# haberdashPI/SignalOperators.jl

Hardware: NVIDIA B200
Metric: sink Msamples/s (Filt+resample+Mix chain) at 1/2/4/8 B200; % of HBM peak (higher is better)
Workload: dtype f64

## Files before the change

signaloperators.jl_b200/csrc/k_fir_tmap.cuh:

```cuda
#pragma once
#include <cuda.h>

#include <type_traits>

#include "k_fir_mma.cuh"

namespace sigops {

constexpr int kFtRows = 128;
constexpr int kFtSlotPos = 16;
constexpr int kFtSlotBytes = kFtRows * 128;
constexpr int kFtMaxSlots = 10;
constexpr int kFtNCW = 8, kFtNAW = 4;
constexpr int kFtThreads = 16 * 32;
constexpr int kFtRegsCompute = 176, kFtRegsHelper = 112, kFtRegsMisc = 40;
constexpr int kFtMaxKs = 64;

struct FirTmParams {
    double* scalars;
    int nscalars, sumsq_slot, nch;
    int64_t nrows, n_out;
    int tapsper;
    int ks;
    int nslot;
    int64_t ntiles, tiles_per_seg;
    const double* pfb;
    const double* dpfb;
    const int64_t* xi0;
    const int32_t* poff;
    const double* alpha;
    int tab_doubles;
    double gain;
    const double* bands_g;
    int period_tiles;
    int64_t epoch_tiles;
    int n_epochs;
    long long* dbg;
    int exp;
};

inline size_t fir_tm_smem_bytes(int nslot, int ks, int tab_doubles, bool has_dpfb) {
    return (size_t)nslot * kFtSlotBytes + 2 * 16384 + (size_t)2 * 4 * ks * 8 * sizeof(double) +
           (size_t)tab_doubles * sizeof(double) * (has_dpfb ? 2 : 1) + 1024;
}

__device__ __forceinline__ void tmap_load_2d(unsigned smem_dst, const CUtensorMap* tm, int c0, int c1, uint64_t* bar) {
    asm volatile("cp.async.bulk.tensor.2d.shared::cluster.global.mbarrier::complete_tx::bytes [%0], [%1, {%2, %3}], [%4];" ::"r"(smem_dst),
                 "l"(tm), "r"(c0), "r"(c1), "r"(smem_u32(bar))
                 : "memory");
}
__device__ __forceinline__ void tmap_store_2d(const CUtensorMap* tm, int c0, int c1, unsigned smem_src) {
    asm volatile("cp.async.bulk.tensor.2d.global.shared::cta.bulk_group [%0, {%1, %2}], [%3];" ::"l"(tm), "r"(c0), "r"(c1), "r"(smem_src)
                 : "memory");
}
__device__ __forceinline__ double lds_f64(unsigned a) {
    double v;
    asm volatile("ld.shared.f64 %0, [%1];" : "=d"(v) : "r"(a));
    return v;
}
__device__ __forceinline__ void sts_f64(unsigned a, double v) { asm volatile("st.shared.f64 [%0], %1;" ::"r"(a), "d"(v) : "memory"); }
__device__ __forceinline__ void sts_v2f64(unsigned a, double x, double y) {
    asm volatile("st.shared.v2.f64 [%0], {%1, %2};" ::"r"(a), "d"(x), "d"(y) : "memory");
}

__device__ __forceinline__ void mbar_wait_a(unsigned bar, unsigned parity) {
    asm volatile(
        "{\n"
        ".reg .pred p;\n"
        "LAB_WAIT:\n"
        "mbarrier.try_wait.parity.shared::cta.b64 p, [%0], %1;\n"
        "@p bra LAB_DONE;\n"
        "bra LAB_WAIT;\n"
        "LAB_DONE:\n"
        "}\n" ::"r"(bar), "r"(parity) : "memory");
}
__device__ __forceinline__ void mbar_arrive_a(unsigned bar) {
    asm volatile("mbarrier.arrive.shared::cta.b64 _, [%0];" ::"r"(bar) : "memory");
}

template <bool SSQ, bool DBG = false>
__global__ void __launch_bounds__(kFtThreads, 1)
k_fir_tmap(const __grid_constant__ FirTmParams P, const __grid_constant__ CUtensorMap tm_in,
           const __grid_constant__ CUtensorMap tm_out) {
    extern __shared__ unsigned char ft_smem_raw[];
    __shared__ uint64_t bar_full[kFtMaxSlots], bar_done[4], bar_taps[2], bar_stg_full[2], bar_stg_free[2];
    __shared__ unsigned done_count;

    const unsigned ring = (smem_u32(ft_smem_raw) + 1023u) & ~1023u;
    const unsigned stg = ring + (unsigned)P.nslot * kFtSlotBytes;
    const unsigned bands = stg + 2 * 16384;
    const unsigned tabs = bands + 2u * 4u * (unsigned)P.ks * 64u;

    const int tid = threadIdx.x, warp = tid >> 5, lane = tid & 31;
    const int row0 = (int)blockIdx.y * kFtRows;
    const int64_t t0 = (int64_t)blockIdx.x * P.tiles_per_seg;
    const int64_t t1 = (t0 + P.tiles_per_seg < P.ntiles) ? t0 + P.tiles_per_seg : P.ntiles;
    if (t0 >= t1) return;

    for (int i = tid; i < P.tab_doubles; i += kFtThreads) {
        sts_f64(tabs + 8u * i, __ldg(P.pfb + i) * P.gain);
        if (P.dpfb) sts_f64(tabs + 8u * (P.tab_doubles + i), __ldg(P.dpfb + i) * P.gain);
    }
    if (tid == 0) {
        done_count = 0u;
        for (int i = 0; i < P.nslot; ++i) mbar_init(&bar_full[i], 1);
        for (int i = 0; i < 4; ++i) mbar_init(&bar_done[i], kFtNCW);
        mbar_init(&bar_taps[0], P.bands_g ? 2 : kFtNAW * 32);
        mbar_init(&bar_taps[1], P.bands_g ? 2 : kFtNAW * 32);
        for (int i = 0; i < 2; ++i) {
            mbar_init(&bar_stg_full[i], kFtNCW / 2);
            mbar_init(&bar_stg_free[i], 1);
        }
        asm volatile("fence.mbarrier_init.release.cluster;" ::: "memory");
    }
    fence_async_smem();
    __syncthreads();

    const int64_t pos_base = (__ldg(P.xi0 + t0 * kFmT) - P.tapsper + 1) & ~int64_t(kFtSlotPos - 1);
    const unsigned band_tile = 4u * (unsigned)P.ks * 64u;

    if (warp < kFtNCW) {
        constexpr int F = 8;
        const int gw = warp & 3, rw = warp >> 2;
        asm volatile("setmaxnreg.inc.sync.aligned.u32 %0;" ::"n"(kFtRegsCompute));
        const int kk = lane & 3, rr = lane >> 2;
        const int rmap = ((rr & 1) << 2) | (rr & 2) | (rr >> 2);
        const int rloc = rw * (8 * F) + rmap;
        const int nn = rr ^ ((kk >> 1) << 2);
        unsigned key = (unsigned)rmap << 4;
        unsigned srow = stg + rloc * 128;
        unsigned bcol = (unsigned)((gw * P.ks + kk) * 64 + nn * 8);
        unsigned arow1 = ring + rloc * 128;
        unsigned ring_end = arow1 + (unsigned)P.nslot * kFtSlotBytes;
        unsigned a_taps = smem_u32(&bar_taps[0]), a_free = smem_u32(&bar_stg_free[rw]), a_full = smem_u32(&bar_stg_full[rw]);
        unsigned a_done = smem_u32(&bar_done[0]), a_cnt = smem_u32(&done_count), lead = lane == 0 ? 1u : 0u;
        asm volatile("" : "+r"(key), "+r"(srow), "+r"(bcol), "+r"(arow1), "+r"(ring_end));
        asm volatile("" : "+r"(a_taps), "+r"(a_free), "+r"(a_full), "+r"(a_done), "+r"(a_cnt), "+r"(lead));
        const int nt = (int)(t1 - t0);
        const int64_t* xp = P.xi0 + t0 * kFmT + 8 * gw;
        double ssq[SSQ ? 8 : 1];
#pragma unroll
        for (int i = 0; i < (SSQ ? 8 : 1); ++i) ssq[i] = 0.0;

        int64_t xq_nx, x7_nx;
        auto fetch_idx = [&](int u) {
            xq_nx = __ldg(xp + (int64_t)u * kFmT);
            x7_nx = __ldg(xp + (int64_t)u * kFmT + 7);
        };
        fetch_idx(0);
        long long dbg_acc[5] = {0, 0, 0, 0, 0};

        unsigned cur = arow1, nxt = arow1;
        int jcur = 0;
        unsigned off[4];
        bool w[4];
        unsigned bq = 0;
        int nbt = 0;
        struct Ops { double a[F], b; };
        Ops o0, o1;

        auto load_ops = [&](Ops& o, auto J) {
            const unsigned ap = (w[J.value] ? nxt : cur) + off[J.value];
#pragma unroll
            for (int i = 0; i < F; ++i) o.a[i] = lds_f64(ap + i * 1024);
            o.b = lds_f64(bq);
            bq += 256;
        };
        auto next_slot = [&]() {
            ++jcur;
            cur = nxt;
            nxt += kFtSlotBytes;
            if (nxt == ring_end) nxt = arow1;
        };
        auto setup = [&](int u, Ops& o) {
            const long long cs = DBG ? clock64() : 0;
            const int s = u & 1;
            const int r = (int)(xq_nx - P.tapsper + 1 - pos_base) + kk;
            int n = (int)(x7_nx - xq_nx) + P.tapsper + 3;
            n >>= 2;
            nbt = n < (P.ks >> 2) ? n : (P.ks >> 2);
            if (u + 1 < nt) fetch_idx(u + 1);
            const int j_new = r >> 4;
            int slot = (int)((cur - arow1) / kFtSlotBytes) + (j_new - jcur);
            while (slot >= P.nslot) slot -= P.nslot;
            while (slot < 0) slot += P.nslot;
            jcur = j_new;
            cur = arow1 + (unsigned)slot * kFtSlotBytes;
            nxt = cur + kFtSlotBytes;
            if (nxt == ring_end) nxt = arow1;
            const unsigned sub0 = (unsigned)(r & 15) << 3;
#pragma unroll
            for (int J = 0; J < 4; ++J) {
                const unsigned q = sub0 + 32u * J;
                w[J] = q >= 128u;
                off[J] = (q & 127u) ^ key;
            }
            bq = bands + s * band_tile + bcol;
            const long long c0 = DBG ? clock64() : 0;
            if (!(P.exp & 16)) mbar_wait_a(a_taps + 8u * s, (unsigned)(u >> 1) & 1u);
            if (DBG) dbg_acc[0] += clock64() - c0;
            load_ops(o, std::integral_constant<int, 0>{});
            if (DBG) dbg_acc[1] += clock64() - cs;
        };
        auto mma_block = [&](double (&acc)[F][2], const Ops& o) {
#pragma unroll
            for (int i = 0; i < F; ++i) dmma884(acc[i][0], acc[i][1], o.a[i], o.b);
        };
        auto stage_store = [&](double (&o)[F][2], int u_old) {
            const long long c0 = DBG ? clock64() : 0;
            if (u_old > 0) mbar_wait_a(a_free, (unsigned)(u_old - 1) & 1u);
            if (DBG) dbg_acc[2] += clock64() - c0;
            if (!(P.exp & 1)) {
                const unsigned sp = srow + (gw >> 1) * 16384 + ((unsigned)(((gw & 1) * 4 + kk) << 4) ^ key);
#pragma unroll
                for (int i = 0; i < F; ++i) sts_v2f64(sp + i * 1024, o[i][0], o[i][1]);
            }
            if (SSQ) {
#pragma unroll
                for (int i = 0; i < F; ++i) ssq[i] = fma(o[i][0], o[i][0], fma(o[i][1], o[i][1], ssq[i]));
            }
            if (DBG) dbg_acc[3] += clock64() - c0;
        };
        auto stage_signal = [&]() {
            const long long c0 = DBG ? clock64() : 0;
            fence_async_smem();
            __syncwarp();
            if (lead) mbar_arrive_a(a_full);
            if (DBG) dbg_acc[3] += clock64() - c0;
        };
        auto tile = [&](double (&acc)[F][2], double (&old)[F][2], int u) {
            const bool more = u + 1 < nt;
#pragma unroll
            for (int i = 0; i < F; ++i) acc[i][0] = acc[i][1] = 0.0;
            const int n = nbt;
            using I0 = std::integral_constant<int, 0>;
            using I1 = std::integral_constant<int, 1>;
            using I2 = std::integral_constant<int, 2>;
            using I3 = std::integral_constant<int, 3>;
            int b = 0;
            bool signalled = u == 0;
            while (true) {
                if (b + 1 < n) {
                    load_ops(o1, I1{});
                    mma_block(acc, o0);
                    if (b == 0 && u > 0) stage_store(old, u - 1);
                } else {
                    if (more) setup(u + 1, o1);
                    mma_block(acc, o0);
                    if (b == 0 && u > 0) stage_store(old, u - 1);
                    o0 = o1;
                    break;
                }
                ++b;
                if (b + 1 < n) {
                    load_ops(o0, I2{});
                    mma_block(acc, o1);
                } else {
                    if (more) setup(u + 1, o0);
                    mma_block(acc, o1);
                    break;
                }
                ++b;
                if (b + 1 < n) {
                    load_ops(o1, I3{});
                    mma_block(acc, o0);
                    if (b == 2 && u > 0) { stage_signal(); signalled = true; }
                } else {
                    if (more) setup(u + 1, o1);
                    mma_block(acc, o0);
                    o0 = o1;
                    break;
                }
                ++b;
                if (b + 1 < n) {
                    next_slot();
                    load_ops(o0, I0{});
                    mma_block(acc, o1);
                } else {
                    if (more) setup(u + 1, o0);
                    mma_block(acc, o1);
                    break;
                }
                ++b;
            }
            if (!signalled) stage_signal();
            __syncwarp();
            if (lead) {
                mbar_arrive_a(a_done + 8u * (u & 3));
                asm volatile("red.release.cta.shared::cta.add.u32 [%0], 1;" ::"r"(a_cnt) : "memory");
            }
        };

        double accA[F][2], accB[F][2];
        setup(0, o0);
        const long long cstart = DBG ? clock64() : 0;
        for (int u = 0; u < nt; u += 2) {
            tile(accA, accB, u);
            if (u + 1 < nt) tile(accB, accA, u + 1);
        }
        if (DBG && warp == 0 && lane == 0) {
            long long* d = P.dbg + ((size_t)blockIdx.y * gridDim.x + blockIdx.x) * 8;
            d[0] = dbg_acc[0]; d[1] = dbg_acc[1]; d[2] = dbg_acc[2]; d[3] = clock64() - cstart; d[6] = dbg_acc[3];
        }
        if (nt & 1) stage_store(accA, nt - 1);
        else stage_store(accB, nt - 1);
        stage_signal();
        if (SSQ) {
#pragma unroll
            for (int i = 0; i < F; ++i) {
                double v = ssq[i];
                v += __shfl_xor_sync(0xffffffffu, v, 1);
                v += __shfl_xor_sync(0xffffffffu, v, 2);
                const int64_t row = (int64_t)row0 + rloc + 8 * i;
                if (kk == 0 && row < P.nrows) atomicAdd(P.scalars + (size_t)(row / P.nch) * P.nscalars + P.sumsq_slot, v);
            }
        }
    } else if (warp < kFtNCW + kFtNAW) {
        asm volatile("setmaxnreg.dec.sync.aligned.u32 %0;" ::"n"(kFtRegsHelper));
        const int grp = warp - kFtNCW;
        if (P.bands_g) {
            if (grp == 0 && lane == 0) {
                const unsigned bytes = 4u * (unsigned)P.ks * 64u;
                int64_t jwait = 0;
                int jw_slot = 0;
                unsigned jw_par = 0;
                for (int64_t t = t0; t < t1; ++t) {
                    const int64_t u = t - t0;
                    const int s = (int)(u & 1);
                    const int64_t hi = (__ldg(P.xi0 + t * kFmT + kFmT - 1) + 4 - pos_base + (kFtSlotPos - 1)) >> 4;
                    if (u >= 2) mbar_wait(&bar_done[(u - 2) & 3], (unsigned)((u - 2) >> 2) & 1u);
                    mbar_expect_tx(&bar_taps[s], bytes);
                    int64_t ep = t / P.epoch_tiles;
                    ep = ep < P.n_epochs ? ep : P.n_epochs - 1;
                    const double* src = P.bands_g + (size_t)(ep * P.period_tiles + t % P.period_tiles) * (bytes / 8);
                    asm volatile("cp.async.bulk.shared::cluster.global.mbarrier::complete_tx::bytes [%0], [%1], %2, [%3];" ::"r"(
                                     bands + (unsigned)s * band_tile),
                                 "l"(src), "r"(bytes), "r"(smem_u32(&bar_taps[s]))
                                 : "memory");
                    while (jwait < hi && !(P.exp & 8)) {
                        mbar_wait(&bar_full[jw_slot], jw_par);
                        ++jwait;
                        if (++jw_slot == P.nslot) { jw_slot = 0; jw_par ^= 1u; }
                    }
                    mbar_arrive(&bar_taps[s]);
                }
            }
            return;
        }
        const int kk = lane & 3, rr = lane >> 2;
        const unsigned pf_tab = tabs, dpf_tab = tabs + 8u * P.tab_doubles;
        const bool has_d = P.dpfb != nullptr;
        const int nblk = P.ks >> 3;
        long long hdbg[2] = {0, 0};
        int64_t jwait = 0;
        int jw_slot = 0;
        unsigned jw_par = 0;
        int64_t xe_nx = __ldg(P.xi0 + t0 * kFmT + kFmT - 1);
        int64_t xi_nx = __ldg(P.xi0 + t0 * kFmT + 8 * grp + (lane & 7));
        int po_nx = __ldg(P.poff + t0 * kFmT + 8 * grp + (lane & 7));
        double al_nx = __ldg(P.alpha + t0 * kFmT + 8 * grp + (lane & 7));
        for (int64_t t = t0; t < t1; ++t) {
            const int64_t u = t - t0;
            const int s = (int)(u & 1);
            const int64_t m = t * kFmT + 8 * grp + (lane & 7);
            const int64_t xi = xi_nx;
            const bool live = m < P.n_out;
            const int po = po_nx;
            const double al = live ? al_nx : 0.0;
            const int64_t hi = (xe_nx + 4 - pos_base + (kFtSlotPos - 1)) >> 4;
            if (t + 1 < t1) {
                xi_nx = __ldg(P.xi0 + m + kFmT);
                po_nx = __ldg(P.poff + m + kFmT);
                al_nx = __ldg(P.alpha + m + kFmT);
                xe_nx = __ldg(P.xi0 + (t + 1) * kFmT + kFmT - 1);
            }
            const int64_t xg = __shfl_sync(0xffffffffu, xi, 0);
            const int st = live ? (int)(xi - xg) : (1 << 20);
            const int st_c0 = __shfl_sync(0xffffffffu, st, 2 * kk), st_c1 = __shfl_sync(0xffffffffu, st, 2 * kk + 1);
            const int po_c0 = __shfl_sync(0xffffffffu, po, 2 * kk), po_c1 = __shfl_sync(0xffffffffu, po, 2 * kk + 1);
            const int st_a0 = __shfl_sync(0xffffffffu, st, kk), st_a1 = __shfl_sync(0xffffffffu, st, 4 + kk);
            const int po_a0 = __shfl_sync(0xffffffffu, po, kk), po_a1 = __shfl_sync(0xffffffffu, po, 4 + kk);
            const double al_b = __shfl_sync(0xffffffffu, al, rr);
            const double b0v = (kk == rr) ? al_b : 0.0, b1v = (4 + kk == rr) ? al_b : 0.0;
            const unsigned band = bands + s * band_tile + (unsigned)(grp * P.ks) * 64u;
            const long long c0 = DBG ? clock64() : 0;
            if (u >= 2) mbar_wait(&bar_done[(u - 2) & 3], (unsigned)((u - 2) >> 2) & 1u);
            const long long c1 = DBG ? clock64() : 0;
            if (DBG) hdbg[0] += c1 - c0;
            for (int b0 = 0; b0 < ((P.exp & 4) ? 0 : nblk); b0 += 4) {
                double cv0[4], cv1[4], a0[4], a1[4];
#pragma unroll
                for (int i = 0; i < 4; ++i) {
                    const int k = 8 * (b0 + i) + rr;
                    const bool on = b0 + i < nblk;
                    const unsigned tc0 = (unsigned)(k - st_c0), tc1 = (unsigned)(k - st_c1);
                    const unsigned ta0 = (unsigned)(k - st_a0), ta1 = (unsigned)(k - st_a1);
                    cv0[i] = on && tc0 < (unsigned)P.tapsper ? lds_f64(pf_tab + 8u * ((unsigned)po_c0 + tc0)) : 0.0;
                    cv1[i] = on && tc1 < (unsigned)P.tapsper ? lds_f64(pf_tab + 8u * ((unsigned)po_c1 + tc1)) : 0.0;
                    a0[i] = has_d && on && ta0 < (unsigned)P.tapsper ? lds_f64(dpf_tab + 8u * ((unsigned)po_a0 + ta0)) : 0.0;
                    a1[i] = has_d && on && ta1 < (unsigned)P.tapsper ? lds_f64(dpf_tab + 8u * ((unsigned)po_a1 + ta1)) : 0.0;
                }
                if (has_d) {
#pragma unroll
                    for (int i = 0; i < 4; ++i)
                        if (b0 + i < nblk) dmma884(cv0[i], cv1[i], a0[i], b0v);
#pragma unroll
                    for (int i = 0; i < 4; ++i)
                        if (b0 + i < nblk) dmma884(cv0[i], cv1[i], a1[i], b1v);
                }
#pragma unroll
                for (int i = 0; i < 4; ++i) {
                    const int k = 8 * (b0 + i) + rr;
                    if (b0 + i < nblk) sts_v2f64(band + 8u * (unsigned)(k * 8 + ((2 * kk) ^ (((k >> 1) & 1) << 2))), cv0[i], cv1[i]);
                }
            }
            while (jwait < hi && !(P.exp & 8)) {
                mbar_wait(&bar_full[jw_slot], jw_par);
                ++jwait;
                if (++jw_slot == P.nslot) { jw_slot = 0; jw_par ^= 1u; }
            }
            mbar_arrive(&bar_taps[s]);
            if (DBG) hdbg[1] += clock64() - c1;
        }
        if (DBG && grp == 0 && lane == 0) {
            long long* d = P.dbg + ((size_t)blockIdx.y * gridDim.x + blockIdx.x) * 8;
            d[4] = hdbg[0]; d[5] = hdbg[1];
        }
    } else {
      asm volatile("setmaxnreg.dec.sync.aligned.u32 %0;" ::"n"(kFtRegsMisc));
      if (warp == kFtNCW + kFtNAW) {
        if (lane == 0 && !(P.exp & 8)) {
            const int64_t last_need = __ldg(P.xi0 + (t1 - 1) * kFmT + kFmT - 1) + 4;
            const int64_t nslots_total = (last_need - pos_base + (kFtSlotPos - 1)) >> 4;
            auto lo_of = [&](int64_t t) { return (__ldg(P.xi0 + t * kFmT) - P.tapsper + 1 - pos_base) >> 4; };
            int64_t tp = t0;
            int64_t lo_next = t0 + 1 < t1 ? lo_of(t0 + 1) : (int64_t(1) << 62);
            int s = 0;
            for (int64_t j = 0; j < nslots_total; ++j) {
                if (j >= P.nslot) {
                    const int64_t k = j - P.nslot;
                    while (lo_next <= k) {
                        ++tp;
                        lo_next = tp + 1 < t1 ? lo_of(tp + 1) : (int64_t(1) << 62);
                    }
                    const unsigned target = (unsigned)(tp - t0 + 1) * kFtNCW;
                    unsigned seen;
                    while (true) {
                        asm volatile("ld.acquire.cta.shared::cta.u32 %0, [%1];" : "=r"(seen) : "r"(smem_u32(&done_count)) : "memory");
                        if (seen >= target) break;
                        if (P.exp & 32) __nanosleep(64);
                    }
                }
                mbar_expect_tx(&bar_full[s], kFtSlotBytes);
                tmap_load_2d(ring + (unsigned)s * kFtSlotBytes, &tm_in, (int)(pos_base + j * kFtSlotPos), row0, &bar_full[s]);
                if (++s == P.nslot) s = 0;
            }
        }
      } else {
        const int h = warp - (kFtNCW + kFtNAW + 1);
        if (h < 2 && lane == 0) {
            const bool rows_live = (int64_t)row0 + 64 * h < P.nrows;
            for (int64_t t = t0; t < t1; ++t) {
                const int64_t u = t - t0;
                mbar_wait(&bar_stg_full[h], (unsigned)u & 1u);
                const int64_t m0 = t * kFmT;
                if (!(P.exp & 2) && rows_live) {
                    tmap_store_2d(&tm_out, (int)m0, row0 + 64 * h, stg + 8192u * h);
                    if (m0 + 16 < P.n_out) tmap_store_2d(&tm_out, (int)(m0 + 16), row0 + 64 * h, stg + 16384 + 8192u * h);
                }
                bulk_commit();
                bulk_wait_read_all();
                mbar_arrive(&bar_stg_free[h]);
            }
            bulk_wait_all();
        }
      }
    }
}

}
```

signaloperators.jl_b200/csrc/runtime.cu:

```cuda
#include <algorithm>
#include <array>
#include <atomic>
#include <chrono>
#include <cmath>
#include <cstdarg>
#include <cstdio>
#include <cstdlib>
#include <cstring>
#include <functional>
#include <future>
#include <unordered_map>
#include <memory>
#include <mutex>
#include <string>
#include <thread>
#include <vector>

#include <cuda_runtime.h>

#include "../../include/signalops.h"
#include "common.h"
#include "launchers.h"
#include "k_iir_carry.cuh"
#include "k_fir.cuh"
// ... 157 lines not shown
struct FirDerived {
    std::vector<int64_t> xi0;
    std::vector<double> phi;
    std::vector<int32_t> poff;
    std::vector<double> alpha;
    int dpad = 0, pmax = 0;
    int pmax32 = 0;
    int ring32 = 0;
    int in_buf = -1;
    int64_t in_len = 0;
    bool epi_const = true;
    double epi_scale = 1.0;
    int64_t period = 0;
    int64_t epoch_tiles = 0;
    int64_t n_epochs = 0;
};

struct StageRT {
    sigops_stage st;
    IirDerived iir;
    FirDerived fir;
};

struct PlanDev {
    bool ready = false;
    sigops_instr* instrs = nullptr;
    double* blob = nullptr;
    std::vector<int64_t*> xi0;
    std::vector<double*> phi;
    std::vector<int32_t*> poff;
    std::vector<double*> alpha;
    std::unordered_map<uint64_t, double*> carry;
    std::unordered_map<uint64_t, double*> bands;
};

}

struct sigops_ctx {
    std::vector<Device> devs;
    std::string err;
    std::mutex mu;
    size_t ws_budget = size_t(16) << 30;
    bool profiling = false;
};

struct sigops_plan {
    sigops_ctx* ctx = nullptr;
    sigops_plan_header h{};
    std::vector<sigops_bufdesc> bufs;
    std::vector<sigops_tabledesc> tables;
    std::vector<sigops_instr> instrs;
    std::vector<sigops_piece> pieces;
    std::vector<StageRT> stages;
    std::vector<double> blob;
    std::vector<PlanDev> dev;
    int nbuf() const { return (int)bufs.size(); }
    int max_stack = 0;
    bool has_randn = false;
    uint64_t uid = 0;
};

namespace {


int program_stack_depth(const sigops_plan& p, int start, int len, bool allow_stage, const char* what) {
    if (len < 0 || start < 0 || (size_t)start + len > p.instrs.size())
// ... 466 lines not shown
    d.phi.assign(p.stages.size(), nullptr);
    d.poff.assign(p.stages.size(), nullptr);
    d.alpha.assign(p.stages.size(), nullptr);
    for (size_t i = 0; i < p.stages.size(); ++i) {
        const FirDerived& f = p.stages[i].fir;
        if (p.stages[i].st.kind != SIGOPS_STAGE_FIR) continue;
        CUDA_OK(cudaMalloc(&d.xi0[i], f.xi0.size() * sizeof(int64_t)));
        CUDA_OK(cudaMalloc(&d.phi[i], f.phi.size() * sizeof(double)));
        CUDA_OK(cudaMemcpy(d.xi0[i], f.xi0.data(), f.xi0.size() * sizeof(int64_t), cudaMemcpyHostToDevice));
        CUDA_OK(cudaMemcpy(d.phi[i], f.phi.data(), f.phi.size() * sizeof(double), cudaMemcpyHostToDevice));
        CUDA_OK(cudaMalloc(&d.poff[i], f.poff.size() * sizeof(int32_t)));
        CUDA_OK(cudaMalloc(&d.alpha[i], f.alpha.size() * sizeof(double)));
        CUDA_OK(cudaMemcpy(d.poff[i], f.poff.data(), f.poff.size() * sizeof(int32_t), cudaMemcpyHostToDevice));
        CUDA_OK(cudaMemcpy(d.alpha[i], f.alpha.data(), f.alpha.size() * sizeof(double), cudaMemcpyHostToDevice));
    }
    d.ready = true;
}

void free_plan_dev(sigops_plan& p) {
    for (size_t di = 0; di < p.dev.size(); ++di) {
        PlanDev& d = p.dev[di];
        if (!d.ready) continue;
        cudaSetDevice(p.ctx->devs[di].ordinal);
        cudaFree(d.instrs);
        cudaFree(d.blob);
        for (auto q : d.xi0) cudaFree(q);
        for (auto q : d.phi) cudaFree(q);
        for (auto q : d.poff) cudaFree(q);
        for (auto q : d.alpha) cudaFree(q);
        for (auto& kv : d.carry) cudaFree(kv.second);
        d.carry.clear();
        for (auto& kv : d.bands) cudaFree(kv.second);
        d.bands.clear();
        d.ready = false;
    }
}


struct IirLaunch {
    int blocks_per_row;
    int64_t L, Wc, nchunks;
    bool need_matrix;
    double cost = 0.0;
};

IirLaunch choose_iir_chunking_flat(const StageRT& s, int64_t rows, int sm_count, bool allow_matrix = true) {
    const int64_t N = s.st.n_out;
    const int64_t W64 = round_up(std::max<int64_t>(s.iir.W, 1), kStageCols);
    const int64_t jmax = std::max<int64_t>(1, (N + kStageCols - 1) / kStageCols);
    double best = 1e300;
    int64_t bestL = kStageCols * jmax;
    const int64_t step = std::max<int64_t>(1, jmax / 4096);
    for (int64_t j = 1; j <= jmax; j += step) {
        const int64_t L = j * kStageCols;
        const int64_t cpr = (N + L - 1) / L;
        const bool matrix = cpr > 1 && W64 >= L;
        if (matrix && !allow_matrix && j + step <= jmax) continue;
        const int64_t blocks = (((rows * cpr) + 31) / 32 + kTmaWarps - 1) / kTmaWarps;
        const int64_t waves = (blocks + sm_count - 1) / sm_count;
        double cost;
        if (matrix) cost = (double)waves * (2.0 * (double)L + 1200.0) + 3.0 * (double)cpr + 400.0;
        else cost = (double)waves * ((double)L + (cpr > 1 ? (double)W64 : 0.0) + 600.0);
        if (N % L) cost *= 1.02;
        if (cost < best) { best = cost; bestL = L; }
    }
    IirLaunch r;
// ... 128 lines not shown
}

const double* period_bands(const Wave& w, int ks) {
    const uint64_t key = ((uint64_t)w.si << 16) | (uint64_t)ks;
    auto it = w.pd.bands.find(key);
    if (it != w.pd.bands.end()) return it->second;
    const sigops_plan& p = w.p;
    const StageRT& s = p.stages[w.si];
    const sigops_stage& g = s.st;
    const int64_t Pp = s.fir.period;
    const double* hp = p.blob.data() + p.tables[g.pfb_table].offset;
    const double* hd = g.dpfb_table >= 0 ? p.blob.data() + p.tables[g.dpfb_table].offset : nullptr;
    const size_t per_epoch = (size_t)(Pp / 8) * ks * 8;
    std::vector<double> tab(per_epoch * (size_t)s.fir.n_epochs, 0.0);
    for (int64_t e = 0; e < s.fir.n_epochs; ++e) {
        const int64_t start = e * s.fir.epoch_tiles * kFmT;
        for (int64_t q = 0; q < Pp; ++q) {
            const int64_t m = start + q, m0 = m & ~int64_t(7);
            const int n = (int)(m - m0), stn = (int)(s.fir.xi0[m] - s.fir.xi0[m0]);
            double* band = tab.data() + per_epoch * (size_t)e + (size_t)((q & ~int64_t(7)) / 8) * ks * 8;
            for (int t = 0; t < g.taps_per_phase && stn + t < ks; ++t) {
                const double pf = hp[s.fir.poff[m] + t] * s.fir.epi_scale;
                const double h = hd ? std::fma(hd[s.fir.poff[m] + t] * s.fir.epi_scale, s.fir.alpha[m], pf) : pf;
                const int k = stn + t;
                band[k * 8 + (n ^ (((k >> 1) & 1) << 2))] = h;
            }
        }
    }
    double* dptr = nullptr;
    CUDA_OK(cudaMalloc(&dptr, tab.size() * sizeof(double)));
    CUDA_OK(cudaMemcpy(dptr, tab.data(), tab.size() * sizeof(double), cudaMemcpyHostToDevice));
    w.pd.bands.emplace(key, dptr);
    return dptr;
}

std::array<double, 8> fir_cycles_per_tile(cudaStream_t stream, size_t nblocks, int64_t tiles_per_seg,
                                          const std::function<void(long long*)>& launch) {
    long long* dbg = nullptr;
    CUDA_OK(cudaMalloc(&dbg, nblocks * 8 * sizeof(long long)));
    CUDA_OK(cudaMemset(dbg, 0, nblocks * 8 * sizeof(long long)));
    launch(dbg);
    CUDA_OK(cudaStreamSynchronize(stream));
    std::vector<long long> h(nblocks * 8);
    CUDA_OK(cudaMemcpy(h.data(), dbg, h.size() * sizeof(long long), cudaMemcpyDeviceToHost));
    cudaFree(dbg);
    std::array<double, 8> sum{};
    for (size_t b = 0; b < nblocks; ++b)
        for (int k = 0; k < 8; ++k) sum[k] += (double)h[b * 8 + k];
    const double per = 1.0 / ((double)nblocks * (double)tiles_per_seg);
    for (double& v : sum) v *= per;
    return sum;
}

template <class... P, class... A>
void launch_dyn_smem(void (*kernel)(P...), dim3 grid, int threads, size_t smem, cudaStream_t st, const A&... args) {
    ensure_dyn_smem(kernel, smem);
    kernel<<<grid, threads, smem, st>>>(args...);
}

void plan_map_stage(const Wave& w) {
    const sigops_plan& p = w.p;
    const sigops_stage& g = p.stages[w.si].st;
    MapParams P{};
    P.instrs = w.pd.instrs; P.bufrefs = w.d_refs; P.scalars = w.scalars; P.inst0 = w.inst0;
    P.nbuf = w.nbuf; P.nscalars = w.nscal;
    P.out_buf = g.out_buf; P.sumsq_slot = g.sumsq_slot; P.out_nch = p.bufs[g.out_buf].nchannels;
// ... 163 lines not shown
        else launch_iir_generic(LAUNCH_FIX, M_, grid, stack_iir, st, P);
    });
}

bool plan_fir_tmap(const Wave& w, const FirParams& P) {
    const StageRT& s = w.p.stages[w.si];
    const sigops_stage& g = s.st;
    const int64_t rows = P.nrows;
    if (rows <= 64 || getenv("SIGOPS_NO_FIR_TMAP") || !iir_tmap_available() || rows >= (int64_t(1) << 31) ||
        g.n_out >= (int64_t(1) << 31) || s.fir.in_len >= (int64_t(1) << 31))
        return false;
    const int ks = (int)round_up(s.fir.dpad + g.taps_per_phase, 8);
    const int win_slots = (s.fir.pmax32 + 3 + 14) / 16 + 1;
    const bool has_d = P.dpfb != nullptr;
    const double* bands_g = nullptr;
    int period_tiles = 0;
    if (s.fir.period > 0 && g.sumsq_slot < 0 && !getenv("SIGOPS_NO_FIR_BANDS") &&
        (size_t)(s.fir.period / 8) * ks * 64 * (size_t)s.fir.n_epochs <= (size_t(96) << 20)) {
        bands_g = period_bands(w, ks);
        period_tiles = (int)(s.fir.period / kFmT);
    }
    const int64_t tabd = bands_g ? 0 : (int64_t)g.n_phases * g.taps_per_phase;
    int nslot = kFtMaxSlots;
    while (nslot > win_slots + 1 && fir_tm_smem_bytes(nslot, ks, (int)tabd, has_d) > kFirTmSmemLimit) --nslot;
    char *bin = nullptr, *bout = nullptr;
    int64_t sin_ = 0, sout = 0;
    TensorMapBlob mi, mo;
    if (!(ks <= kFtMaxKs && nslot >= win_slots + 1 && fir_tm_smem_bytes(nslot, ks, (int)tabd, has_d) <= kFirTmSmemLimit &&
          strided_matrix(w.refs, w.ninst, w.nbuf, s.fir.in_buf, 8, SIGOPS_F64, &bin, &sin_) &&
          strided_matrix(w.refs, w.ninst, w.nbuf, g.out_buf, 8, SIGOPS_F64, &bout, &sout) && s.fir.in_len >= 1 &&
          tmap_encode_2d_f64(&mi, bin, s.fir.in_len, rows, sin_, kFtSlotPos, kFtRows) &&
          tmap_encode_2d_f64(&mo, bout, g.n_out, rows, sout, 16, kFtRows / 2)))
        return false;
    FirTmParams T{};
    T.scalars = w.scalars; T.nscalars = w.nscal; T.sumsq_slot = g.sumsq_slot; T.nch = g.nchannels;
    T.nrows = rows; T.n_out = g.n_out; T.tapsper = g.taps_per_phase; T.ks = ks; T.nslot = nslot;
    T.ntiles = (g.n_out + kFmT - 1) / kFmT;
    T.pfb = P.pfb; T.dpfb = P.dpfb; T.xi0 = P.xi0; T.poff = w.pd.poff[w.si]; T.alpha = w.pd.alpha[w.si];
    T.tab_doubles = (int)tabd;
    T.bands_g = bands_g; T.period_tiles = period_tiles;
    T.epoch_tiles = s.fir.epoch_tiles; T.n_epochs = (int)s.fir.n_epochs;
    T.gain = s.fir.epi_scale;
    if (const char* e = getenv("SIGOPS_FIR_EXP")) T.exp = atoi(e);
    const int64_t groups = (rows + kFtRows - 1) / kFtRows;
    if (groups > 65535) return false;
    T.tiles_per_seg = choose_tiles_per_segment(T.ntiles, groups, w.sm_count);
    const int64_t nseg = (T.ntiles + T.tiles_per_seg - 1) / T.tiles_per_seg;
    const size_t smem = fir_tm_smem_bytes(nslot, ks, (int)tabd, has_d);
    dim3 tgrid((unsigned)nseg, (unsigned)groups);
    if (getenv("SIGOPS_DEBUG")) {
        fprintf(stderr, "[sigops] FIR stage %zu: tensor-map rows=%lld n_out=%lld taps=%d ks=%d slots=%d (window %d) grid=%lldx%lld tiles/seg=%lld smem=%zu gain=%g period=%lld outputs%s\n",
                w.si, (long long)rows, (long long)g.n_out, T.tapsper, ks, nslot, win_slots, (long long)nseg, (long long)groups,
                (long long)T.tiles_per_seg, smem, T.gain, (long long)s.fir.period, bands_g ? " (tap bands from the period tables)" : "");
        if (bands_g) fprintf(stderr, "[sigops]   %lld epochs of %lld tiles\n", (long long)s.fir.n_epochs, (long long)s.fir.epoch_tiles);
    }
    if (getenv("SIGOPS_FIR_DBG")) {
        const auto c = fir_cycles_per_tile(w.stream, (size_t)nseg * groups, T.tiles_per_seg, [&](long long* dbg) {
            FirTmParams D = T;
            D.dbg = dbg;
            launch_dyn_smem(k_fir_tmap<false, true>, tgrid, kFtThreads, smem, w.stream, D, *(const CUtensorMap*)&mi,
                            *(const CUtensorMap*)&mo);
        });
        fprintf(stderr, "[sigops] FIR tmap cycles/tile  compute: set-up %.0f (of it wait_taps %.0f) staging %.0f (of it wait_stg %.0f) total %.0f | helper: wait_done %.0f build %.0f\n",
                c[1], c[0], c[6], c[2], c[3], c[4], c[5]);
    }
    const auto kernel = g.sumsq_slot >= 0 ? k_fir_tmap<true> : k_fir_tmap<false>;
    w.add(KIND_FIR, [=](cudaStream_t st) {
        launch_dyn_smem(kernel, tgrid, kFtThreads, smem, st, T, *(const CUtensorMap*)&mi, *(const CUtensorMap*)&mo);
    });
    return true;
}

bool plan_fir_mma(const Wave& w, const FirParams& P) {
    const StageRT& s = w.p.stages[w.si];
    const sigops_stage& g = s.st;
    const int64_t rows = P.nrows;
    FirMmaParams Q{};
    Q.bufrefs = w.d_refs; Q.scalars = w.scalars; Q.nbuf = w.nbuf; Q.nscalars = w.nscal;
    Q.in_buf = s.fir.in_buf; Q.out_buf = g.out_buf; Q.sumsq_slot = g.sumsq_slot;
    Q.in_len = s.fir.in_len; Q.nch = g.nchannels; Q.nrows = rows; Q.n_out = g.n_out;
    Q.tapsper = g.taps_per_phase;
    Q.ks = (int)round_up(s.fir.dpad + g.taps_per_phase, 4);
    Q.ring = s.fir.ring32;
    Q.pitch = Q.ring + ((4 - Q.ring % 16) + 16) % 16;
    Q.pfb = P.pfb; Q.dpfb = P.dpfb; Q.xi0 = P.xi0; Q.poff = w.pd.poff[w.si]; Q.alpha = w.pd.alpha[w.si];
    Q.ntiles = (g.n_out + kFmT - 1) / kFmT;
    Q.gain = s.fir.epi_scale;
    const int64_t tabd = (int64_t)g.n_phases * g.taps_per_phase;
    const size_t tab_bytes = (size_t)tabd * 8 * (P.dpfb ? 2 : 1);
    Q.tab_doubles = (int)tabd;
    if (tab_bytes > 48 * 1024) return false;
    auto smem_for = [&](int RBx) {
        return (size_t)RBx * Q.pitch * 8 + (size_t)2 * 4 * Q.ks * kFmHbPitch * 8 + tab_bytes;
    };
    int RB = rows > 64 ? 128 : (rows > 32 ? 64 : 32);
    while (RB > 32 && smem_for(RB) > kFirMmaSmemLimit) RB >>= 1;
    const int64_t groups = (rows + RB - 1) / RB;
// ... 876 lines not shown
```

Measured before the change: 275,100.

## Split tap and done barriers per column group and replace shared counter with per-warp progress

Barriers for band taps and tile completion are split per column group, so each compute group waits only on its own helper warp and its own band slice. The bands-from-global path is spread over four helper warps, each issuing a smaller bulk copy for its group. The single atomic done counter becomes per-warp progress slots that the TMA producer reduces with a min scan, and it now always backs off with nanosleep. Polling waits on producer and store warps use try_wait with a suspend-time hint to cut issue pressure on shared memory. In exchange there are more barriers and more bulk copies, and the producer's scan over eight slots may add latency.

```diff
diff --git a/signaloperators.jl_b200/csrc/k_fir_tmap.cuh b/signaloperators.jl_b200/csrc/k_fir_tmap.cuh
--- a/signaloperators.jl_b200/csrc/k_fir_tmap.cuh
+++ b/signaloperators.jl_b200/csrc/k_fir_tmap.cuh
@@ -74,6 +74,17 @@
         "LAB_DONE:\n"
         "}\n" ::"r"(bar), "r"(parity) : "memory");
 }
+__device__ __forceinline__ void mbar_wait_idle(uint64_t* bar, unsigned parity) {
+    asm volatile(
+        "{\n"
+        ".reg .pred p;\n"
+        "LAB_WAIT:\n"
+        "mbarrier.try_wait.parity.shared::cta.b64 p, [%0], %1, %2;\n"
+        "@p bra LAB_DONE;\n"
+        "bra LAB_WAIT;\n"
+        "LAB_DONE:\n"
+        "}\n" ::"r"(smem_u32(bar)), "r"(parity), "r"(1000000u) : "memory");
+}
 __device__ __forceinline__ void mbar_arrive_a(unsigned bar) {
     asm volatile("mbarrier.arrive.shared::cta.b64 _, [%0];" ::"r"(bar) : "memory");
 }
@@ -83,8 +94,8 @@
 k_fir_tmap(const __grid_constant__ FirTmParams P, const __grid_constant__ CUtensorMap tm_in,
            const __grid_constant__ CUtensorMap tm_out) {
     extern __shared__ unsigned char ft_smem_raw[];
-    __shared__ uint64_t bar_full[kFtMaxSlots], bar_done[4], bar_taps[2], bar_stg_full[2], bar_stg_free[2];
-    __shared__ unsigned done_count;
+    __shared__ uint64_t bar_full[kFtMaxSlots], bar_done[4][4], bar_taps[4][2], bar_stg_full[2], bar_stg_free[2];
+    __shared__ unsigned done_tiles[kFtNCW];
 
     const unsigned ring = (smem_u32(ft_smem_raw) + 1023u) & ~1023u;
     const unsigned stg = ring + (unsigned)P.nslot * kFtSlotBytes;
@@ -102,11 +113,13 @@
         if (P.dpfb) sts_f64(tabs + 8u * (P.tab_doubles + i), __ldg(P.dpfb + i) * P.gain);
     }
     if (tid == 0) {
-        done_count = 0u;
+        for (int i = 0; i < kFtNCW; ++i) done_tiles[i] = 0u;
         for (int i = 0; i < P.nslot; ++i) mbar_init(&bar_full[i], 1);
-        for (int i = 0; i < 4; ++i) mbar_init(&bar_done[i], kFtNCW);
-        mbar_init(&bar_taps[0], P.bands_g ? 2 : kFtNAW * 32);
-        mbar_init(&bar_taps[1], P.bands_g ? 2 : kFtNAW * 32);
+        for (int g = 0; g < 4; ++g) {
+            for (int i = 0; i < 4; ++i) mbar_init(&bar_done[g][i], kFtNCW / 4);
+            mbar_init(&bar_taps[g][0], P.bands_g ? 2 : 32);
+            mbar_init(&bar_taps[g][1], P.bands_g ? 2 : 32);
+        }
         for (int i = 0; i < 2; ++i) {
             mbar_init(&bar_stg_full[i], kFtNCW / 2);
             mbar_init(&bar_stg_free[i], 1);
@@ -132,8 +145,8 @@
         unsigned bcol = (unsigned)((gw * P.ks + kk) * 64 + nn * 8);
         unsigned arow1 = ring + rloc * 128;
         unsigned ring_end = arow1 + (unsigned)P.nslot * kFtSlotBytes;
-        unsigned a_taps = smem_u32(&bar_taps[0]), a_free = smem_u32(&bar_stg_free[rw]), a_full = smem_u32(&bar_stg_full[rw]);
-        unsigned a_done = smem_u32(&bar_done[0]), a_cnt = smem_u32(&done_count), lead = lane == 0 ? 1u : 0u;
+        unsigned a_taps = smem_u32(&bar_taps[gw][0]), a_free = smem_u32(&bar_stg_free[rw]), a_full = smem_u32(&bar_stg_full[rw]);
+        unsigned a_done = smem_u32(&bar_done[gw][0]), a_cnt = smem_u32(&done_tiles[warp]), lead = lane == 0 ? 1u : 0u;
         asm volatile("" : "+r"(key), "+r"(srow), "+r"(bcol), "+r"(arow1), "+r"(ring_end));
         asm volatile("" : "+r"(a_taps), "+r"(a_free), "+r"(a_full), "+r"(a_done), "+r"(a_cnt), "+r"(lead));
         const int nt = (int)(t1 - t0);
@@ -287,7 +300,7 @@
             __syncwarp();
             if (lead) {
                 mbar_arrive_a(a_done + 8u * (u & 3));
-                asm volatile("red.release.cta.shared::cta.add.u32 [%0], 1;" ::"r"(a_cnt) : "memory");
+                asm volatile("st.release.cta.shared::cta.u32 [%0], %1;" ::"r"(a_cnt), "r"(u + 1) : "memory");
             }
         };
 
@@ -319,8 +332,8 @@
         asm volatile("setmaxnreg.dec.sync.aligned.u32 %0;" ::"n"(kFtRegsHelper));
         const int grp = warp - kFtNCW;
         if (P.bands_g) {
-            if (grp == 0 && lane == 0) {
-                const unsigned bytes = 4u * (unsigned)P.ks * 64u;
+            if (lane == 0) {
+                const unsigned bytes = (unsigned)P.ks * 64u;
                 int64_t jwait = 0;
                 int jw_slot = 0;
                 unsigned jw_par = 0;
@@ -328,21 +341,21 @@
                     const int64_t u = t - t0;
                     const int s = (int)(u & 1);
                     const int64_t hi = (__ldg(P.xi0 + t * kFmT + kFmT - 1) + 4 - pos_base + (kFtSlotPos - 1)) >> 4;
-                    if (u >= 2) mbar_wait(&bar_done[(u - 2) & 3], (unsigned)((u - 2) >> 2) & 1u);
-                    mbar_expect_tx(&bar_taps[s], bytes);
+                    if (u >= 2) mbar_wait_idle(&bar_done[grp][(u - 2) & 3], (unsigned)((u - 2) >> 2) & 1u);
+                    mbar_expect_tx(&bar_taps[grp][s], bytes);
                     int64_t ep = t / P.epoch_tiles;
                     ep = ep < P.n_epochs ? ep : P.n_epochs - 1;
-                    const double* src = P.bands_g + (size_t)(ep * P.period_tiles + t % P.period_tiles) * (bytes / 8);
+                    const double* src = P.bands_g + (size_t)(ep * P.period_tiles + t % P.period_tiles) * (4 * bytes / 8) + grp * (bytes / 8);
                     asm volatile("cp.async.bulk.shared::cluster.global.mbarrier::complete_tx::bytes [%0], [%1], %2, [%3];" ::"r"(
-                                     bands + (unsigned)s * band_tile),
-                                 "l"(src), "r"(bytes), "r"(smem_u32(&bar_taps[s]))
+                                     bands + (unsigned)s * band_tile + (unsigned)grp * bytes),
+                                 "l"(src), "r"(bytes), "r"(smem_u32(&bar_taps[grp][s]))
                                  : "memory");
                     while (jwait < hi && !(P.exp & 8)) {
-                        mbar_wait(&bar_full[jw_slot], jw_par);
+                        mbar_wait_idle(&bar_full[jw_slot], jw_par);
                         ++jwait;
                         if (++jw_slot == P.nslot) { jw_slot = 0; jw_par ^= 1u; }
                     }
-                    mbar_arrive(&bar_taps[s]);
+                    mbar_arrive(&bar_taps[grp][s]);
                 }
             }
             return;
@@ -384,7 +397,7 @@
             const double b0v = (kk == rr) ? al_b : 0.0, b1v = (4 + kk == rr) ? al_b : 0.0;
             const unsigned band = bands + s * band_tile + (unsigned)(grp * P.ks) * 64u;
             const long long c0 = DBG ? clock64() : 0;
-            if (u >= 2) mbar_wait(&bar_done[(u - 2) & 3], (unsigned)((u - 2) >> 2) & 1u);
+            if (u >= 2) mbar_wait(&bar_done[grp][(u - 2) & 3], (unsigned)((u - 2) >> 2) & 1u);
             const long long c1 = DBG ? clock64() : 0;
             if (DBG) hdbg[0] += c1 - c0;
             for (int b0 = 0; b0 < ((P.exp & 4) ? 0 : nblk); b0 += 4) {
@@ -419,7 +432,7 @@
                 ++jwait;
                 if (++jw_slot == P.nslot) { jw_slot = 0; jw_par ^= 1u; }
             }
-            mbar_arrive(&bar_taps[s]);
+            mbar_arrive(&bar_taps[grp][s]);
             if (DBG) hdbg[1] += clock64() - c1;
         }
         if (DBG && grp == 0 && lane == 0) {
@@ -443,12 +456,17 @@
                         ++tp;
                         lo_next = tp + 1 < t1 ? lo_of(tp + 1) : (int64_t(1) << 62);
                     }
-                    const unsigned target = (unsigned)(tp - t0 + 1) * kFtNCW;
-                    unsigned seen;
+                    const unsigned target = (unsigned)(tp - t0 + 1);
                     while (true) {
-                        asm volatile("ld.acquire.cta.shared::cta.u32 %0, [%1];" : "=r"(seen) : "r"(smem_u32(&done_count)) : "memory");
+                        unsigned seen = ~0u;
+#pragma unroll
+                        for (int i = 0; i < kFtNCW; ++i) {
+                            unsigned v;
+                            asm volatile("ld.acquire.cta.shared::cta.u32 %0, [%1];" : "=r"(v) : "r"(smem_u32(&done_tiles[i])) : "memory");
+                            seen = v < seen ? v : seen;
+                        }
                         if (seen >= target) break;
-                        if (P.exp & 32) __nanosleep(64);
+                        __nanosleep(64);
                     }
                 }
                 mbar_expect_tx(&bar_full[s], kFtSlotBytes);
@@ -462,7 +480,7 @@
             const bool rows_live = (int64_t)row0 + 64 * h < P.nrows;
             for (int64_t t = t0; t < t1; ++t) {
                 const int64_t u = t - t0;
-                mbar_wait(&bar_stg_full[h], (unsigned)u & 1u);
+                mbar_wait_idle(&bar_stg_full[h], (unsigned)u & 1u);
                 const int64_t m0 = t * kFmT;
                 if (!(P.exp & 2) && rows_live) {
                     tmap_store_2d(&tm_out, (int)m0, row0 + 64 * h, stg + 8192u * h);
```

Result: no change. 275,300 (median of 6 runs) (+0.1%).

## Precompute per-tile FIR schedule table and streamline compute-warp tile loop

Applied to the files above, without the earlier changes.

Adds a host-built per-tile table (first input position and block count per group, plus the tile's end position) in 32-bit ints. The compute, helper and loader warps read it instead of the 64-bit xi0 indices, which removes per-tile index arithmetic, the division-based slot lookup and the while-loop wraparound. The compute loop now zero-initialises accumulators through the first MMA (C=0) rather than with an explicit clear, and issues the done-signal and next-tile index prefetch earlier. The path falls back to the old kernel when positions exceed the int32 range or the slot advance is too large, and the table costs a one-time upload per stage.

```diff
diff --git a/signaloperators.jl_b200/csrc/k_fir_tmap.cuh b/signaloperators.jl_b200/csrc/k_fir_tmap.cuh
--- a/signaloperators.jl_b200/csrc/k_fir_tmap.cuh
+++ b/signaloperators.jl_b200/csrc/k_fir_tmap.cuh
@@ -15,6 +15,13 @@
 constexpr int kFtThreads = 16 * 32;
 constexpr int kFtRegsCompute = 176, kFtRegsHelper = 112, kFtRegsMisc = 40;
 constexpr int kFtMaxKs = 64;
+
+struct alignas(16) FtTile {
+    int2 grp[4];
+    int end;
+    int pad_[3];
+};
+static_assert(sizeof(FtTile) == 48, "FtTile is read as int2 / int by the kernel");
 
 struct FirTmParams {
     double* scalars;
@@ -27,6 +34,7 @@
     const double* pfb;
     const double* dpfb;
     const int64_t* xi0;
+    const FtTile* tiles;
     const int32_t* poff;
     const double* alpha;
     int tab_doubles;
@@ -61,6 +69,11 @@
 __device__ __forceinline__ void sts_f64(unsigned a, double v) { asm volatile("st.shared.f64 [%0], %1;" ::"r"(a), "d"(v) : "memory"); }
 __device__ __forceinline__ void sts_v2f64(unsigned a, double x, double y) {
     asm volatile("st.shared.v2.f64 [%0], {%1, %2};" ::"r"(a), "d"(x), "d"(y) : "memory");
+}
+
+__device__ __forceinline__ void dmma884_z(double& d0, double& d1, double a, double b) {
+    asm volatile("mma.sync.aligned.m8n8k4.row.col.f64.f64.f64.f64 {%0,%1}, {%2}, {%3}, {%4,%4};"
+                 : "=d"(d0), "=d"(d1) : "d"(a), "d"(b), "d"(0.0));
 }
 
 __device__ __forceinline__ void mbar_wait_a(unsigned bar, unsigned parity) {
@@ -116,7 +129,7 @@
     fence_async_smem();
     __syncthreads();
 
-    const int64_t pos_base = (__ldg(P.xi0 + t0 * kFmT) - P.tapsper + 1) & ~int64_t(kFtSlotPos - 1);
+    const int pos_base = __ldg(&P.tiles[t0].grp[0].x) & ~(kFtSlotPos - 1);
     const unsigned band_tile = 4u * (unsigned)P.ks * 64u;
 
     if (warp < kFtNCW) {
@@ -134,24 +147,25 @@
         unsigned ring_end = arow1 + (unsigned)P.nslot * kFtSlotBytes;
         unsigned a_taps = smem_u32(&bar_taps[0]), a_free = smem_u32(&bar_stg_free[rw]), a_full = smem_u32(&bar_stg_full[rw]);
         unsigned a_done = smem_u32(&bar_done[0]), a_cnt = smem_u32(&done_count), lead = lane == 0 ? 1u : 0u;
-        asm volatile("" : "+r"(key), "+r"(srow), "+r"(bcol), "+r"(arow1), "+r"(ring_end));
+        int kpos = kk - pos_base;
+        asm volatile("" : "+r"(key), "+r"(srow), "+r"(bcol), "+r"(arow1), "+r"(ring_end), "+r"(kpos));
         asm volatile("" : "+r"(a_taps), "+r"(a_free), "+r"(a_full), "+r"(a_done), "+r"(a_cnt), "+r"(lead));
         const int nt = (int)(t1 - t0);
-        const int64_t* xp = P.xi0 + t0 * kFmT + 8 * gw;
+        const int2* tp = &P.tiles[t0].grp[gw];
         double ssq[SSQ ? 8 : 1];
 #pragma unroll
         for (int i = 0; i < (SSQ ? 8 : 1); ++i) ssq[i] = 0.0;
 
-        int64_t xq_nx, x7_nx;
+        int2 rec_nx;
         auto fetch_idx = [&](int u) {
-            xq_nx = __ldg(xp + (int64_t)u * kFmT);
-            x7_nx = __ldg(xp + (int64_t)u * kFmT + 7);
+            const int2* a = tp + (u < nt ? u : nt - 1) * (int)(sizeof(FtTile) / sizeof(int2));
+            asm volatile("ld.global.nc.v2.s32 {%0, %1}, [%2];" : "=r"(rec_nx.x), "=r"(rec_nx.y) : "l"(a));
         };
         fetch_idx(0);
         long long dbg_acc[5] = {0, 0, 0, 0, 0};
 
         unsigned cur = arow1, nxt = arow1;
-        int jcur = 0;
+        int jfirst = 0, sfirst = 0;
         unsigned off[4];
         bool w[4];
         unsigned bq = 0;
@@ -167,7 +181,6 @@
             bq += 256;
         };
         auto next_slot = [&]() {
-            ++jcur;
             cur = nxt;
             nxt += kFtSlotBytes;
             if (nxt == ring_end) nxt = arow1;
@@ -175,16 +188,13 @@
         auto setup = [&](int u, Ops& o) {
             const long long cs = DBG ? clock64() : 0;
             const int s = u & 1;
-            const int r = (int)(xq_nx - P.tapsper + 1 - pos_base) + kk;
-            int n = (int)(x7_nx - xq_nx) + P.tapsper + 3;
-            n >>= 2;
-            nbt = n < (P.ks >> 2) ? n : (P.ks >> 2);
-            if (u + 1 < nt) fetch_idx(u + 1);
+            const int r = rec_nx.x + kpos;
+            nbt = rec_nx.y;
             const int j_new = r >> 4;
-            int slot = (int)((cur - arow1) / kFtSlotBytes) + (j_new - jcur);
-            while (slot >= P.nslot) slot -= P.nslot;
-            while (slot < 0) slot += P.nslot;
-            jcur = j_new;
+            int slot = sfirst + (j_new - jfirst);
+            if (slot >= P.nslot) slot -= P.nslot;
+            jfirst = j_new;
+            sfirst = slot;
             cur = arow1 + (unsigned)slot * kFtSlotBytes;
             nxt = cur + kFtSlotBytes;
             if (nxt == ring_end) nxt = arow1;
@@ -198,13 +208,19 @@
             bq = bands + s * band_tile + bcol;
             const long long c0 = DBG ? clock64() : 0;
             if (!(P.exp & 16)) mbar_wait_a(a_taps + 8u * s, (unsigned)(u >> 1) & 1u);
-            if (DBG) dbg_acc[0] += clock64() - c0;
+            const long long c1 = DBG ? clock64() : 0;
             load_ops(o, std::integral_constant<int, 0>{});
-            if (DBG) dbg_acc[1] += clock64() - cs;
-        };
-        auto mma_block = [&](double (&acc)[F][2], const Ops& o) {
-#pragma unroll
-            for (int i = 0; i < F; ++i) dmma884(acc[i][0], acc[i][1], o.a[i], o.b);
+            if (DBG) {
+                dbg_acc[0] += c1 - c0;
+                dbg_acc[1] += clock64() - cs - (c1 - c0);
+            }
+        };
+        auto mma_block = [&](double (&acc)[F][2], const Ops& o, auto first) {
+#pragma unroll
+            for (int i = 0; i < F; ++i) {
+                if (first.value) dmma884_z(acc[i][0], acc[i][1], o.a[i], o.b);
+                else dmma884(acc[i][0], acc[i][1], o.a[i], o.b);
+            }
         };
         auto stage_store = [&](double (&o)[F][2], int u_old) {
             const long long c0 = DBG ? clock64() : 0;
@@ -226,48 +242,58 @@
             fence_async_smem();
             __syncwarp();
             if (lead) mbar_arrive_a(a_full);
-            if (DBG) dbg_acc[3] += clock64() - c0;
+            if (DBG) dbg_acc[4] += clock64() - c0;
+        };
+        auto last_block = [&](int u, int n, Ops& o) {
+            const long long c0 = DBG ? clock64() : 0;
+            __syncwarp();
+            if (lead) {
+                mbar_arrive_a(a_done + 8u * (u & 3));
+                asm volatile("red.release.cta.shared::cta.add.u32 [%0], 1;" ::"r"(a_cnt) : "memory");
+            }
+            if (DBG) dbg_acc[4] += clock64() - c0;
+            if (n <= 3) fetch_idx(u + 1);
+            if (u + 1 < nt) setup(u + 1, o);
         };
         auto tile = [&](double (&acc)[F][2], double (&old)[F][2], int u) {
-            const bool more = u + 1 < nt;
-#pragma unroll
-            for (int i = 0; i < F; ++i) acc[i][0] = acc[i][1] = 0.0;
             const int n = nbt;
             using I0 = std::integral_constant<int, 0>;
             using I1 = std::integral_constant<int, 1>;
             using I2 = std::integral_constant<int, 2>;
             using I3 = std::integral_constant<int, 3>;
-            int b = 0;
+            using First = std::true_type;
+            using Acc = std::false_type;
             bool signalled = u == 0;
-            while (true) {
-                if (b + 1 < n) {
-                    load_ops(o1, I1{});
-                    mma_block(acc, o0);
-                    if (b == 0 && u > 0) stage_store(old, u - 1);
-                } else {
-                    if (more) setup(u + 1, o1);
-                    mma_block(acc, o0);
-                    if (b == 0 && u > 0) stage_store(old, u - 1);
-                    o0 = o1;
-                    break;
-                }
-                ++b;
+            if (1 < n) {
+                load_ops(o1, I1{});
+                mma_block(acc, o0, First{});
+                if (u > 0) stage_store(old, u - 1);
+            } else {
+                last_block(u, n, o1);
+                mma_block(acc, o0, First{});
+                if (u > 0) stage_store(old, u - 1);
+                o0 = o1;
+            }
+            for (int b = 1; b < n; ++b) {
                 if (b + 1 < n) {
                     load_ops(o0, I2{});
-                    mma_block(acc, o1);
+                    mma_block(acc, o1, Acc{});
                 } else {
-                    if (more) setup(u + 1, o0);
-                    mma_block(acc, o1);
+                    last_block(u, n, o0);
+                    mma_block(acc, o1, Acc{});
                     break;
                 }
                 ++b;
                 if (b + 1 < n) {
                     load_ops(o1, I3{});
-                    mma_block(acc, o0);
-                    if (b == 2 && u > 0) { stage_signal(); signalled = true; }
+                    mma_block(acc, o0, Acc{});
+                    if (b == 2) {
+                        if (u > 0) { stage_signal(); signalled = true; }
+                        fetch_idx(u + 1);
+                    }
                 } else {
-                    if (more) setup(u + 1, o1);
-                    mma_block(acc, o0);
+                    last_block(u, n, o1);
+                    mma_block(acc, o0, Acc{});
                     o0 = o1;
                     break;
                 }
@@ -275,20 +301,24 @@
                 if (b + 1 < n) {
                     next_slot();
                     load_ops(o0, I0{});
-                    mma_block(acc, o1);
+                    mma_block(acc, o1, Acc{});
                 } else {
-                    if (more) setup(u + 1, o0);
-                    mma_block(acc, o1);
+                    last_block(u, n, o0);
+                    mma_block(acc, o1, Acc{});
                     break;
                 }
                 ++b;
+                if (b + 1 < n) {
+                    load_ops(o1, I1{});
+                    mma_block(acc, o0, Acc{});
+                } else {
+                    last_block(u, n, o1);
+                    mma_block(acc, o0, Acc{});
+                    o0 = o1;
+                    break;
+                }
             }
             if (!signalled) stage_signal();
-            __syncwarp();
-            if (lead) {
-                mbar_arrive_a(a_done + 8u * (u & 3));
-                asm volatile("red.release.cta.shared::cta.add.u32 [%0], 1;" ::"r"(a_cnt) : "memory");
-            }
         };
 
         double accA[F][2], accB[F][2];
@@ -301,6 +331,7 @@
         if (DBG && warp == 0 && lane == 0) {
             long long* d = P.dbg + ((size_t)blockIdx.y * gridDim.x + blockIdx.x) * 8;
             d[0] = dbg_acc[0]; d[1] = dbg_acc[1]; d[2] = dbg_acc[2]; d[3] = clock64() - cstart; d[6] = dbg_acc[3];
+            d[7] = dbg_acc[4];
         }
         if (nt & 1) stage_store(accA, nt - 1);
         else stage_store(accB, nt - 1);
@@ -327,7 +358,7 @@
                 for (int64_t t = t0; t < t1; ++t) {
                     const int64_t u = t - t0;
                     const int s = (int)(u & 1);
-                    const int64_t hi = (__ldg(P.xi0 + t * kFmT + kFmT - 1) + 4 - pos_base + (kFtSlotPos - 1)) >> 4;
+                    const int64_t hi = (__ldg(&P.tiles[t].end) - pos_base + (kFtSlotPos - 1)) >> 4;
                     if (u >= 2) mbar_wait(&bar_done[(u - 2) & 3], (unsigned)((u - 2) >> 2) & 1u);
                     mbar_expect_tx(&bar_taps[s], bytes);
                     int64_t ep = t / P.epoch_tiles;
@@ -355,7 +386,7 @@
         int64_t jwait = 0;
         int jw_slot = 0;
         unsigned jw_par = 0;
-        int64_t xe_nx = __ldg(P.xi0 + t0 * kFmT + kFmT - 1);
+        int end_nx = __ldg(&P.tiles[t0].end);
         int64_t xi_nx = __ldg(P.xi0 + t0 * kFmT + 8 * grp + (lane & 7));
         int po_nx = __ldg(P.poff + t0 * kFmT + 8 * grp + (lane & 7));
         double al_nx = __ldg(P.alpha + t0 * kFmT + 8 * grp + (lane & 7));
@@ -367,12 +398,12 @@
             const bool live = m < P.n_out;
             const int po = po_nx;
             const double al = live ? al_nx : 0.0;
-            const int64_t hi = (xe_nx + 4 - pos_base + (kFtSlotPos - 1)) >> 4;
+            const int64_t hi = (end_nx - pos_base + (kFtSlotPos - 1)) >> 4;
             if (t + 1 < t1) {
                 xi_nx = __ldg(P.xi0 + m + kFmT);
                 po_nx = __ldg(P.poff + m + kFmT);
                 al_nx = __ldg(P.alpha + m + kFmT);
-                xe_nx = __ldg(P.xi0 + (t + 1) * kFmT + kFmT - 1);
+                end_nx = __ldg(&P.tiles[t + 1].end);
             }
             const int64_t xg = __shfl_sync(0xffffffffu, xi, 0);
             const int st = live ? (int)(xi - xg) : (1 << 20);
@@ -430,9 +461,8 @@
       asm volatile("setmaxnreg.dec.sync.aligned.u32 %0;" ::"n"(kFtRegsMisc));
       if (warp == kFtNCW + kFtNAW) {
         if (lane == 0 && !(P.exp & 8)) {
-            const int64_t last_need = __ldg(P.xi0 + (t1 - 1) * kFmT + kFmT - 1) + 4;
-            const int64_t nslots_total = (last_need - pos_base + (kFtSlotPos - 1)) >> 4;
-            auto lo_of = [&](int64_t t) { return (__ldg(P.xi0 + t * kFmT) - P.tapsper + 1 - pos_base) >> 4; };
+            const int64_t nslots_total = (__ldg(&P.tiles[t1 - 1].end) - pos_base + (kFtSlotPos - 1)) >> 4;
+            auto lo_of = [&](int64_t t) { return (int64_t)((__ldg(&P.tiles[t].grp[0].x) - pos_base) >> 4); };
             int64_t tp = t0;
             int64_t lo_next = t0 + 1 < t1 ? lo_of(t0 + 1) : (int64_t(1) << 62);
             int s = 0;
diff --git a/signaloperators.jl_b200/csrc/runtime.cu b/signaloperators.jl_b200/csrc/runtime.cu
--- a/signaloperators.jl_b200/csrc/runtime.cu
+++ b/signaloperators.jl_b200/csrc/runtime.cu
@@ -213,6 +213,11 @@
     std::vector<double*> alpha;
     std::unordered_map<uint64_t, double*> carry;
     std::unordered_map<uint64_t, double*> bands;
+    struct TileSchedule {
+        FtTile* dev = nullptr;
+        int max_advance = 0;
+    };
+    std::unordered_map<uint64_t, TileSchedule> tiles;
 };
 
 }
@@ -745,6 +750,8 @@
         d.carry.clear();
         for (auto& kv : d.bands) cudaFree(kv.second);
         d.bands.clear();
+        for (auto& kv : d.tiles) cudaFree(kv.second.dev);
+        d.tiles.clear();
         d.ready = false;
     }
 }
@@ -939,6 +946,38 @@
     CUDA_OK(cudaMemcpy(dptr, tab.data(), tab.size() * sizeof(double), cudaMemcpyHostToDevice));
     w.pd.bands.emplace(key, dptr);
     return dptr;
+}
+
+const PlanDev::TileSchedule& fir_tm_schedule(const Wave& w, int ks) {
+    const uint64_t key = ((uint64_t)w.si << 16) | (uint64_t)ks;
+    auto it = w.pd.tiles.find(key);
+    if (it != w.pd.tiles.end()) return it->second;
+    const StageRT& s = w.p.stages[w.si];
+    const int64_t T = s.st.taps_per_phase, ntiles = (s.st.n_out + kFmT - 1) / kFmT;
+    const std::vector<int64_t>& xi0 = s.fir.xi0;
+    std::vector<FtTile> tab((size_t)ntiles);
+    PlanDev::TileSchedule sched;
+    bool fits = true;
+    int64_t prev_first[4] = {0, 0, 0, 0};
+    for (int64_t t = 0; t < ntiles; ++t) {
+        FtTile& r = tab[(size_t)t];
+        for (int g = 0; g < 4; ++g) {
+            const int64_t m = t * kFmT + 8 * g, first = xi0[m] - T + 1;
+            const int64_t n = std::min<int64_t>((xi0[m + 7] - xi0[m] + T + 3) >> 2, ks >> 2);
+            fits = fits && first >= -(int64_t(1) << 30) && first < (int64_t(1) << 30);
+            r.grp[g] = make_int2((int)first, (int)n);
+            if (t > 0) sched.max_advance = (int)std::max<int64_t>(sched.max_advance, ((first + 3) >> 4) - (prev_first[g] >> 4));
+            prev_first[g] = first;
+        }
+        const int64_t end = xi0[t * kFmT + kFmT - 1] + 4;
+        fits = fits && end + T + 2 * kFtSlotPos < INT32_MAX;
+        r.end = (int)end;
+    }
+    if (fits && ntiles > 0) {
+        CUDA_OK(cudaMalloc(&sched.dev, tab.size() * sizeof(FtTile)));
+        CUDA_OK(cudaMemcpy(sched.dev, tab.data(), tab.size() * sizeof(FtTile), cudaMemcpyHostToDevice));
+    }
+    return w.pd.tiles.emplace(key, sched).first->second;
 }
 
 std::array<double, 8> fir_cycles_per_tile(cudaStream_t stream, size_t nblocks, int64_t tiles_per_seg,
@@ -1168,11 +1207,13 @@
           tmap_encode_2d_f64(&mi, bin, s.fir.in_len, rows, sin_, kFtSlotPos, kFtRows) &&
           tmap_encode_2d_f64(&mo, bout, g.n_out, rows, sout, 16, kFtRows / 2)))
         return false;
+    const PlanDev::TileSchedule& sched = fir_tm_schedule(w, ks);
+    if (!sched.dev || sched.max_advance >= nslot) return false;
     FirTmParams T{};
     T.scalars = w.scalars; T.nscalars = w.nscal; T.sumsq_slot = g.sumsq_slot; T.nch = g.nchannels;
     T.nrows = rows; T.n_out = g.n_out; T.tapsper = g.taps_per_phase; T.ks = ks; T.nslot = nslot;
     T.ntiles = (g.n_out + kFmT - 1) / kFmT;
-    T.pfb = P.pfb; T.dpfb = P.dpfb; T.xi0 = P.xi0; T.poff = w.pd.poff[w.si]; T.alpha = w.pd.alpha[w.si];
+    T.pfb = P.pfb; T.dpfb = P.dpfb; T.xi0 = P.xi0; T.tiles = sched.dev; T.poff = w.pd.poff[w.si]; T.alpha = w.pd.alpha[w.si];
     T.tab_doubles = (int)tabd;
     T.bands_g = bands_g; T.period_tiles = period_tiles;
     T.epoch_tiles = s.fir.epoch_tiles; T.n_epochs = (int)s.fir.n_epochs;
@@ -1197,8 +1238,8 @@
             launch_dyn_smem(k_fir_tmap<false, true>, tgrid, kFtThreads, smem, w.stream, D, *(const CUtensorMap*)&mi,
                             *(const CUtensorMap*)&mo);
         });
-        fprintf(stderr, "[sigops] FIR tmap cycles/tile  compute: set-up %.0f (of it wait_taps %.0f) staging %.0f (of it wait_stg %.0f) total %.0f | helper: wait_done %.0f build %.0f\n",
-                c[1], c[0], c[6], c[2], c[3], c[4], c[5]);
+        fprintf(stderr, "[sigops] FIR tmap cycles/tile  compute: set-up %.0f wait_taps %.0f staging %.0f (of it wait_stg %.0f) signal %.0f total %.0f | helper: wait_done %.0f build %.0f\n",
+                c[1], c[0], c[6], c[2], c[7], c[3], c[4], c[5]);
     }
     const auto kernel = g.sumsq_slot >= 0 ? k_fir_tmap<true> : k_fir_tmap<false>;
     w.add(KIND_FIR, [=](cudaStream_t st) {
```

New measurement: 275,600 before, 279,500 after (median of 6 runs). 1.4% higher.
